# DakeQQ/Audio-Denoiser-ONNX

Measured on AMD Instinct MI355X. Metric: audio_seconds_per_second (GTCRN 16 kHz, batch=256 x 1 s chunks; RTF = 1/value), higher is better.
Workload: dtype f32; 1 GPU; GTCRN 16 kHz, batch=256 x 1 s chunks, fp32, int16 PCM in/out resident in HBM (BASELINE.json configs[1]); chunks_per_gpu=256, chunks_total=256, ranks=1, chunk_samples=16000, out_samples=15872, weights=seeded reference-architecture GTCRN (tests/golden/gtcrn_seed0.adew), stitch_all_gather=False

## Files before the change

audio_denoiser_onnx_amd/csrc/ade_engine.hip:

```cpp
#include "ade_internal.h"
#include "ade_gtcrn_pack.h"

#include "../../include/ade.h"

#if !defined(HIPSIM)
#include <dlfcn.h>
#endif

#include <algorithm>
#include <cmath>
#include <cstdio>
#include <cstdlib>
#include <cstring>
#include <map>
#include <mutex>
#include <string>
#include <vector>

using namespace ade;

namespace {

thread_local std::string g_create_error;

// ... 86 lines not shown
    int* d_ints = nullptr;
    FftTabs tabs{};
    BandTab erb_bm{}, erb_bs{};
    ConvW en0{}, en1{}, de3{}, de4{};
    GtConvW en_gt[3]{}, de_gt[3]{};
    DpW dp[2]{};

    int capacity = 0;
    int last_batch = 0;
    int16_t* d_pcm_in = nullptr;
    int16_t* d_pcm_out = nullptr;
    float* d_f32_out = nullptr;
    float* ws = nullptr;
    float *mean = nullptr, *spec = nullptr, *feat = nullptr, *e0 = nullptr, *e1 = nullptr, *h = nullptr, *zt = nullptr;
    float *xe[3] = {}, *ate[3] = {}, *xd[3] = {}, *atd[3] = {};
    float *rnn = nullptr, *dpm[2] = {}, *dpo[2] = {};
    float *d3 = nullptr, *mask = nullptr, *frames = nullptr;
    int16_t* h_pcm_in = nullptr;
    int16_t* h_pcm_out = nullptr;
    float* h_f32_out = nullptr;

    int stagger_ticks = 2750;
    int wave_swap = 0;
    int seg_prio = 0;
    int xwait_ticks = 20000000;
    int full_taps = 0;
    int xchg_withhold = 0;
    int xwait_retry = 1;
    bool timed_out = false;
    int retries = 0;
    int geometry = -1;
    ade::ChunkFixed* d_fixed = nullptr;
    float* d_xchg = nullptr;
    unsigned* d_xflags = nullptr;
    int* d_xerr = nullptr;
    int xl_B[kXErrWords] = {}, xl_chunk0[kXErrWords] = {};
    int xchg_capacity = 0;
    int xchg_segments = 0;
    bool use_graph = true;
    bool graph_supported = true;
    bool use_fused = true;
    bool use_single = true;
    bool last_fused = false;
    int last_geometry = -1;
    long long* d_clk = nullptr;
    std::vector<GraphEntry> graphs;
// ... 475 lines not shown
        hipEventRecord(e->events[cursor].second, s);
        ++cursor;
        e->events_used = cursor;
    }
};

int pick_geometry(const ade_engine* e, int ) {
    if (e->geometry >= 0) return fused_supported(e->T, e->geometry) ? e->geometry : -1;
    for (int g = fused_geometries() - 1; g >= 0; --g)
        if (fused_supported(e->T, g)) return g;
    return -1;
}

void enqueue(ade_engine* e, hipStream_t s, const int16_t* d_in, int B, int16_t* d_out, float* d_f32, bool prof) {
    const int T = e->T, nfr = B * T;
    Seq q{e, s, prof};
    const View none{nullptr, nullptr};
    const int geo = pick_geometry(e, B);
    const bool fused = e->use_fused && geo >= 0 && !e->gt_sand;
    e->last_fused = fused;
    View x{e->e1, nullptr};
    if (fused) {
        SegPlan plan{};
        plan.nseg = fused_segments(T, geo); plan.xchg = e->d_xchg; plan.flags = e->d_xflags; plan.err = e->d_xerr; plan.wave_swap = e->wave_swap;
        plan.prio = e->seg_prio;
        plan.withhold = e->xchg_withhold;
        plan.wait_ticks = e->xwait_ticks;
        e->last_geometry = geo;
        long long* clk = prof ? e->d_clk : nullptr;
        if (clk) (void)hipMemsetAsync(e->d_clk, 0, kClkSlots * sizeof(long long), s);
        const float* dc = nullptr;
        if (e->n_win > 1) {
            q.begin("pcm_mean"); launch_pcm_mean(s, d_in, B, e->in_len, e->mean, e->n_win); q.end();
            dc = e->mean;
        }
        if (e->use_single && (!prof || e->profile_mode >= 2)) {
            ChunkCall C{};
            C.fixed = e->d_fixed;
            C.dc = dc;
            C.stagger = (geo == 0 && B >= 192) ? e->stagger_ticks : 0;
            C.pcm_in = d_in; C.pcm_out = d_out; C.f32_out = d_f32; C.L = e->in_len; C.T = T; C.B = B;
            C.plan = plan;
            C.full_taps = e->full_taps;
            C.clk = (prof && e->profile_mode == 3) ? e->d_clk : nullptr;
            q.begin("gtcrn_chunk"); launch_gtcrn_chunk(s, geo, C); q.end();
            return;
        }
// ... 631 lines not shown
    d->max_batch = h->capacity / h->n_win;
    d->device = h->device;
    return ADE_OK;
}

ade_status ade_reserve(ade_handle h, int batch) {
    if (!h || batch < 0) return ADE_ERR_BAD_VALUE;
    return reserve(h, batch * h->n_win);
}

ade_status ade_set_option(ade_handle h, const char* key, const char* value) {
    if (!h || !key || !value) return ADE_ERR_BAD_VALUE;
    if (strcmp(key, "stagger_us") == 0) {
        char* end = nullptr;
        const double us = strtod(value, &end);
        if (!value[0] || *end || us < 0.0 || us > 1000.0) return fail(h, ADE_ERR_BAD_VALUE, "option stagger_us: 0..1000");
        h->stagger_ticks = (int)(us * 100.0 + 0.5);
        return ADE_OK;
    }
    if (strcmp(key, "wave_swap") == 0) {
        bool b;
        if (!parse_bool(value, &b)) return fail(h, ADE_ERR_BAD_VALUE, "option wave_swap must be 0/1");
        h->wave_swap = b;
        return ADE_OK;
    }
    if (strcmp(key, "seg_prio") == 0) {
        if (value[0] < '0' || value[0] > '4' || value[1]) return fail(h, ADE_ERR_BAD_VALUE, "option seg_prio: 0..4");
        h->seg_prio = value[0] - '0';
        return ADE_OK;
    }
    if (strcmp(key, "xwait_ms") == 0) {
        char* end = nullptr;
        const double ms = strtod(value, &end);
        if (!value[0] || *end || !(ms >= 0.001) || ms > 20000.0) return fail(h, ADE_ERR_BAD_VALUE, "option xwait_ms: 0.001..20000");
        h->xwait_ticks = (int)(ms * 1e5 + 0.5);
        if (h->sub) h->sub->set_exchange_wait_ticks(h->xwait_ticks);
        free_graphs(h);
        return ADE_OK;
    }
    if (strcmp(key, "pipe_depth") == 0) {
        if (value[0] < '2' || value[0] > '4' || value[1]) return fail(h, ADE_ERR_BAD_VALUE, "option pipe_depth: 2..4");
        for (const auto& sl : h->pipe) if (sl.state == 1) return fail(h, ADE_ERR_BAD_VALUE, "option pipe_depth: submissions are in flight (ade_wait them first)");
        h->pipe_depth = value[0] - '0';
        return ADE_OK;
    }
    if (strcmp(key, "xwait_retry") == 0) {
// ... 306 lines not shown
                    const std::string _what = std::string(#expr) + ": " + hipGetErrorString(_err);                           \
                    if (launched) {                                                                                          \
                        (void)hipStreamSynchronize(h->stream); (void)hipStreamSynchronize(h->s_in); (void)hipStreamSynchronize(h->s_out); \
                        (void)exchange_status(h, "ade_process", false);                                                      \
                        (void)hipGetLastError();                                                                             \
                    }                                                                                                        \
                    return fail(h, ADE_ERR_DEVICE, _what);                                                                   \
                }                                                                                                            \
            } while (0)
            const unsigned epoch = ++h->sio_epoch ? h->sio_epoch : ++h->sio_epoch;
            h->last_batch = rows;
            h->last_fused = true;
            h->last_geometry = geo;
            h->h_sio_epoch[0] = epoch;
            for (int g = 0; g < used; ++g) {
                const int r0 = g * per, nr = std::min(per, rows - r0);
                const size_t i0 = (size_t)r0 * h->in_len;
                const int16_t* src = in + i0;
                if (!in_direct) { memcpy(h->h_pcm_in + i0, in + i0, (size_t)nr * h->in_len * sizeof(int16_t)); src = h->h_pcm_in + i0; }
                SIO_TRY(hipMemcpyAsync(h->d_pcm_in + i0, src, (size_t)nr * h->in_len * sizeof(int16_t), hipMemcpyHostToDevice, h->s_in));
                SIO_TRY(hipMemcpyAsync(h->d_sio_ready + (size_t)g * kReadyStride, h->h_sio_epoch, (size_t)kReadyStride * sizeof(unsigned), hipMemcpyHostToDevice, h->s_in));
                if (g == 0) {
                    ChunkCall C{};
                    C.plan.nseg = fused_segments(h->T, geo); C.plan.xchg = h->d_xchg; C.plan.flags = h->d_xflags; C.plan.err = h->d_xerr; C.plan.wave_swap = h->wave_swap;
                    C.plan.prio = h->seg_prio; C.plan.withhold = h->xchg_withhold; C.plan.wait_ticks = h->xwait_ticks;
                    C.fixed = h->d_fixed;
                    C.pcm_in = h->d_pcm_in; C.pcm_out = h->d_pcm_out; C.f32_out = out_f32 ? h->d_f32_out : nullptr;
                    C.L = h->in_len; C.T = h->T; C.B = rows; C.chunk0 = 0;
                    C.full_taps = h->full_taps;
                    C.in_ready = h->d_sio_ready; C.out_done = h->h_sio_done; C.out_count = h->d_sio_count; C.epoch = epoch; C.group_rows = per;
                    launch_gtcrn_chunk(h->stream, geo, C);
                    launched = true;
                    SIO_TRY(hipGetLastError());
                }
            }
            volatile unsigned* const done = h->h_sio_done;
            bool finished = false;
            for (int g = 0; g < used; ++g) {
                const int r0 = g * per, nr = std::min(per, rows - r0);
                const size_t o0 = (size_t)r0 * h->out_len;
                for (unsigned spins = 0; done[g] != epoch && !finished; ++spins)
                    if ((spins & 0x3ffu) == 0x3ffu && hipStreamQuery(h->stream) == hipSuccess) finished = true;
                if (out_pcm) SIO_TRY(hipMemcpyAsync((pcm_direct ? out_pcm : h->h_pcm_out) + o0, h->d_pcm_out + o0, (size_t)nr * h->out_len * sizeof(int16_t), hipMemcpyDeviceToHost, h->s_out));
                if (out_f32) SIO_TRY(hipMemcpyAsync((f32_direct ? out_f32 : h->h_f32_out) + o0, h->d_f32_out + o0, (size_t)nr * h->out_len * sizeof(float), hipMemcpyDeviceToHost, h->s_out));
            }
#undef SIO_TRY
            (void)hipGetLastError();
// ... 12 lines not shown
        }
    }
    {
        const int geo = pick_geometry(h, rows);
        int n_sub = h->host_split ? h->host_split : (rows >= 128 ? 2 : 1);
        const bool plain = !h->sub && !h->gt_sand && h->use_fused && h->use_single && geo >= 0 && !h->profile && h->n_win == 1;
        if (plain && n_sub > 1 && rows >= 2 * n_sub) {
            const int per = (rows + n_sub - 1) / n_sub;
            h->last_batch = rows;
            h->last_fused = true;
            h->last_geometry = geo;
            const int used = (rows + per - 1) / per;
            for (int k = 0; k < used; ++k) {
                const int r0 = k * per, nr = std::min(per, rows - r0);
                if (!h->sub_streams[k]) HIP_TRY(h, hipStreamCreateWithFlags(&h->sub_streams[k], hipStreamNonBlocking));
                const size_t i0 = (size_t)r0 * h->in_len;
                const int16_t* src = in + i0;
                if (!in_direct) { memcpy(h->h_pcm_in + i0, in + i0, (size_t)nr * h->in_len * sizeof(int16_t)); src = h->h_pcm_in + i0; }
                HIP_TRY(h, hipMemcpyAsync(h->d_pcm_in + i0, src, (size_t)nr * h->in_len * sizeof(int16_t), hipMemcpyHostToDevice, h->sub_streams[k]));
            }
            for (int k = 0; k < used; ++k) {
                const int r0 = k * per, nr = std::min(per, rows - r0);
                ChunkCall C{};
                C.plan.nseg = fused_segments(h->T, geo); C.plan.xchg = h->d_xchg; C.plan.flags = h->d_xflags; C.plan.wave_swap = h->wave_swap;
                C.plan.err = h->d_xerr + k;
                h->xl_B[k] = nr; h->xl_chunk0[k] = r0;
                C.plan.prio = h->seg_prio; C.plan.withhold = r0 == 0 ? h->xchg_withhold : 0; C.plan.wait_ticks = h->xwait_ticks;
                C.fixed = h->d_fixed;
                C.pcm_in = h->d_pcm_in; C.pcm_out = h->d_pcm_out; C.f32_out = out_f32 ? h->d_f32_out : nullptr;
                C.L = h->in_len; C.T = h->T; C.B = nr; C.chunk0 = r0;
                C.full_taps = h->full_taps;
                launch_gtcrn_chunk(h->sub_streams[k], geo, C);
                HIP_TRY(h, hipGetLastError());
            }
            for (int k = 0; k < used; ++k) {
                const int r0 = k * per, nr = std::min(per, rows - r0);
                const size_t o0 = (size_t)r0 * h->out_len;
                hipStream_t s = h->sub_streams[k];
                if (out_pcm) HIP_TRY(h, hipMemcpyAsync((pcm_direct ? out_pcm : h->h_pcm_out) + o0, h->d_pcm_out + o0, (size_t)nr * h->out_len * sizeof(int16_t), hipMemcpyDeviceToHost, s));
                if (out_f32) HIP_TRY(h, hipMemcpyAsync((f32_direct ? out_f32 : h->h_f32_out) + o0, h->d_f32_out + o0, (size_t)nr * h->out_len * sizeof(float), hipMemcpyDeviceToHost, s));
            }
            for (int k = 0; k < used; ++k) HIP_TRY(h, hipStreamSynchronize(h->sub_streams[k]));
            st = exchange_status(h, "ade_process", false);
            for (int k = 0; k < kXErrWords; ++k) h->xl_B[k] = 0;
            if (st != ADE_OK) {
                if (out_pcm && pcm_direct) memset(out_pcm, 0, nout * sizeof(int16_t));
                if (out_f32 && f32_direct) memset(out_f32, 0, nout * sizeof(float));
// ... 639 lines not shown
```

audio_denoiser_onnx_amd/csrc/ade_fused.hip:

```cpp
#include "ade_stage_frontback.h"

namespace ade {

using namespace stage;

namespace {

constexpr size_t cmax(size_t a, size_t b) { return a > b ? a : b; }
template <class G> constexpr size_t chunk_smem_bytes() {
    return cmax(cmax(gt_smem_bytes<G>(), dp_smem_bytes<G>()), cmax(front_smem_bytes<G>(), back_smem_bytes<G>()));
}
static_assert(chunk_smem_bytes<Geo1>() * 2 <= 160 * 1024, "two geometry-1 workgroups must fit one CU's LDS");
static_assert(chunk_smem_bytes<Geo2>() * 4 <= 160 * 1024, "four geometry-2 workgroups must fit one CU's LDS");
static_assert(chunk_smem_bytes<Geo0>() <= 160 * 1024, "geometry 0 must fit one CU's LDS");

__device__ __forceinline__ Seg make_seg(const SegPlan& plan, int B, int T, int block, int& chunk, int chunk0 = 0) {
    const int seg = block / B;
    chunk = chunk0 + block - seg * B;
    const int base = T / plan.nseg, rem = T - base * plan.nseg;
    Seg sg;
    sg.T = T;
    sg.nT = base + (seg < rem ? 1 : 0);
    sg.t0 = seg * base + (seg < rem ? seg : rem);
    sg.prev = seg > 0;
    sg.next = seg + 1 < plan.nseg;
    sg.swap = plan.wave_swap && (seg & 1);
    sg.stream = plan.stream;
    const size_t slot = (size_t)chunk * plan.nseg + seg;
    sg.xo = plan.xchg + slot * kXFloats;
    sg.xi = plan.xchg + (slot - (seg > 0 ? 1 : 0)) * kXFloats;
    sg.fo = plan.flags + slot * kXFlags;
    sg.fi = plan.flags + (slot - (seg > 0 ? 1 : 0)) * kXFlags;
    sg.err = plan.err;
    if (seg == 0 && plan.carry_in) {
        sg.prev = 1;
        sg.xi = plan.carry_in + (size_t)chunk * kXFloats;
        sg.fi = plan.carry_in_flags + (size_t)chunk * kXFlags;
    }
    if (seg + 1 == plan.nseg && plan.carry_out) {
        sg.next = 1;
        sg.xo = plan.carry_out + (size_t)chunk * kXFloats;
        sg.fo = plan.carry_out_flags + (size_t)chunk * kXFlags;
    }
    if (plan.withhold && block == 0) sg.fo = plan.flags + ((size_t)B * plan.nseg - 1) * kXFlags;
    sg.first = !sg.prev;
    sg.base_prio = plan.prio == 4 ? (seg < 2 ? 2 - seg : 0) : (seg > 0 ? plan.prio : 0);
    return sg;
}
__device__ __forceinline__ long long* seg_clk(long long* clk, const Seg& sg, int B, int block) {
// ... 188 lines not shown
```

audio_denoiser_onnx_amd/csrc/ade_internal.h:

```cpp
#pragma once
#include <map>
#include <string>
#include <vector>

#include <hip/hip_runtime.h>

#include <cstddef>
#include <cstdint>

namespace ade {

constexpr int kNfft = 512;
constexpr int kHop = 256;
constexpr int kBins = 257;
constexpr int kBinsPad = 260;
constexpr int kErb = 129;
constexpr int kErbPad = 132;
constexpr int kErbLow = 65;
constexpr int kErbBands = 64;
constexpr int kErbHigh = 192;
constexpr int kF1 = 65;
constexpr int kFw = 33;
constexpr int kCh = 16;
constexpr int kTileFrames = 7;
// ... 88 lines not shown
                         float f32_scale, int nan_to_num );
void launch_half_to_float(hipStream_t s, const uint16_t* in, float* out, long long n);
void launch_float_to_half(hipStream_t s, const float* in, uint16_t* out, long long n);
void launch_ola_pcm_stream(hipStream_t s, const float* frames, float* carry, FftTabs tabs, int B, int T, bool first, int16_t* pcm, float* f32);

constexpr int kXHistFrames = 10;
constexpr int kXHistFloats = 4 * kXHistFrames * kFw * 4;
constexpr int kXTraOff = 6 * kXHistFloats;
constexpr int kXInterOff = kXTraOff + 6 * 16;
constexpr int kXOlaOff = kXInterOff + 2 * kFw * 16;
constexpr int kXPendOff = kXOlaOff + kHop;
constexpr int kXFloats = ((kXPendOff + kHop + 63) / 64) * 64;
constexpr int kXFlags = 16;
constexpr int kXFlagHist = 0, kXFlagTra = 6, kXFlagInter = 12, kXFlagOla = 14;
constexpr int kMaxSegments = 8;
constexpr int kClkSlotsPerSeg = 64 * 10;
struct SegPlan {
    int wait_ticks;
    int nseg;
    float* xchg;
    unsigned* flags;
    int* err;
    int wave_swap;
    float* carry_in;
    unsigned* carry_in_flags;
    float* carry_out;
    unsigned* carry_out_flags;
    int stream;
    int prio;
    int withhold;
};
struct Seg {
    int t0, nT, T;
    int prev, next;
    int swap;
    int stream;
    int first;
    int base_prio;
    float* xo;
    float* xi;
    unsigned* fo;
    unsigned* fi;
    int* err;
};
int fused_geometries();
int fused_max_frames(int geometry);
bool fused_supported(int T, int geometry);
int fused_segments(int T, int geometry);
hipError_t fused_init();
void launch_gtblock(hipStream_t s, int geometry, SegPlan plan, int blk, const float* a, const float* skip, GtConvW w, float* out, int B, int T, long long* clk);
void launch_dpgrnn(hipStream_t s, int geometry, SegPlan plan, int blk, const float* x, DpW w, float* out, int B, int T, long long* clk);
void launch_front(hipStream_t s, int geometry, SegPlan plan, const int16_t* pcm, int B, int L, int T, FftTabs tabs, BandTab erb_bm, ConvW c0, ConvW c1, float* spec,
                  float* e0, float* e1, long long* clk, const float* dc = nullptr);
void launch_back(hipStream_t s, int geometry, SegPlan plan, const float* x, const float* e1, const float* e0, const float* spec, ConvW c3, ConvW c4, BandTab erb_bs,
                 FftTabs tabs, int16_t* pcm, float* f32, int B, int T, long long* clk);

struct ChunkFixed {
    FftTabs tabs;
// ... 85 lines not shown
```

audio_denoiser_onnx_amd/csrc/ade_stage_frontback.h:

```cpp
#pragma once
#include "ade_stage_net.h"

namespace ade {
namespace stage {

constexpr int kWbuf = 264;
constexpr size_t kTabFloats = 512 + 2 * 256 + 2 * 264;
constexpr int kBmCap = 16;
constexpr int kBsCap = 4;

__device__ __forceinline__ float2 rfft_bin(float2 zk, float2 zp, float2 w) {
    const float2 e = make_float2(0.5f * (zk.x + zp.x), 0.5f * (zk.y - zp.y));
    const float2 d = make_float2(0.5f * (zk.x - zp.x), 0.5f * (zk.y + zp.y));
    const float2 o = make_float2(d.y, -d.x);
    return make_float2(e.x + (w.x * o.x - w.y * o.y), e.y + (w.x * o.y + w.y * o.x));
}

struct LdsTabs { const float* win; const float2* tw256; const float2* tw512; };
template <class G>
__device__ __forceinline__ LdsTabs stage_tables(float* dst, const FftTabs& t, int tid) {
    constexpr int kFusedThreads = G::kThreads;
    float* win = dst;
    float* tw256 = dst + 512;
    float* tw512 = tw256 + 512;
// ... 41 lines not shown
            (size_t)(G::kLean ? 0 : kBmCap) * kErbBands + kC0TailW + kC1TailW + 16) * 4;
}

template <class G>
__device__ __forceinline__ void front_stage(float* smem, int chunk, const Seg& sg, const int16_t* __restrict__ pcm, int L, const FftTabs& tabs,
                                            const BandTab& erb, const ConvW& c0, const ConvW& c1, float* __restrict__ spec,
                                            float* __restrict__ e0, float* __restrict__ e1, long long* __restrict__ clk,
                                            const float* __restrict__ dc_rows = nullptr) {
    constexpr int kFusedThreads = G::kThreads, kTileF = G::kTileF, kTileP1 = kTileF * kF1;
    constexpr size_t kFrontFeatFloats = (size_t)kTileF * 3 * kErb;
    constexpr int kGroupShift = (kFusedThreads == 1024 ? 9 : (kFusedThreads == 512 ? 8 : 7));
    static_assert(kFusedThreads == 1024 || kFusedThreads == 512 || kFusedThreads == 256, "front / back conv rounds: 64 lanes per frame");
    constexpr int kBmRows = G::kLean ? 0 : kBmCap;
    const int T = sg.T, tbeg = sg.t0, tend = sg.t0 + sg.nT;
    float2* wbuf_all = reinterpret_cast<float2*>(smem);
    float* feat = smem + kTileF * kWbuf * 2;
    float4* E0 = reinterpret_cast<float4*>(feat + kFrontFeatFloats);
    float* E0f = reinterpret_cast<float*>(E0);
    float* tabmem = reinterpret_cast<float*>(E0 + 4 * kTileP1);
    float* erbw = tabmem + kTabFloats;
    float* w0t = erbw + kBmRows * kErbBands;
    float* w1t = w0t + kC0TailW;
    int* red = reinterpret_cast<int*>(w1t + kC1TailW);
    int tid_ = threadIdx.x;
    ADE_OPAQUE_V(tid_);
    const int tid = tid_, wave = tid >> 6, lane = tid & 63;
    const int16_t* row = pcm + (size_t)chunk * L;
    const int P0 = T * kF1, P = T * kFw;
    float* e0c = e0 + (size_t)chunk * kCh * P0;
    float* e1c = e1 + (size_t)chunk * kCh * P;
    float* specc = spec + (size_t)chunk * T * 2 * kBinsPad;
    ADE_CLK(32);
    const bool pair_ok = ((L & 1) == 0) && ((reinterpret_cast<size_t>(row) & 3) == 0);
    int raw[4];
    const int centre = sg.stream ? 0 : kNfft / 2;
    load_frame_pairs(row, L, tbeg + wave, lane, tbeg + wave < tend, pair_ok, raw, centre);
    const LdsTabs lt = stage_tables<G>(tabmem, tabs, tid);
    const bool erb_lds = erb.count <= kBmRows;
    if (erb_lds)
        for (int i = tid; i < erb.count * kErbBands; i += kFusedThreads) erbw[i] = erb.w[i];
    const int erb_s0 = erb.start[lane];
    for (int i = tid; i < kC0TailW; i += kFusedThreads) w0t[i] = c0.w[i];
    for (int i = tid; i < kC1TailW; i += kFusedThreads) w1t[i] = c1.w[i];
    const float b0t = c0.b[tid & 15], b1t = c1.b[tid & 15];

    if (!dc_rows) {
        int s = 0;
        if (((L & 7) == 0) && ((reinterpret_cast<size_t>(row) & 15) == 0)) {
            const int4* r4 = reinterpret_cast<const int4*>(row);
#pragma unroll 2
            for (int i = tid; i < (L >> 3); i += kFusedThreads) {
                const int4 q = r4[i];
                s += (int)(short)(q.x & 0xffff) + (q.x >> 16) + (int)(short)(q.y & 0xffff) + (q.y >> 16)
                   + (int)(short)(q.z & 0xffff) + (q.z >> 16) + (int)(short)(q.w & 0xffff) + (q.w >> 16);
            }
        } else {
            for (int i = tid; i < L; i += kFusedThreads) s += (int)row[i];
        }
#pragma unroll
        for (int off = 32; off >= 1; off >>= 1) s += __shfl_xor(s, off);
        if (lane == 0) red[wave] = s;
    }
    __syncthreads();
    float dc;
    if (dc_rows) {
        dc = dc_rows[chunk];
    } else {
        long long tot = 0;
#pragma unroll
        for (int i = 0; i < kTileF; ++i) tot += red[i];
        dc = (float)((double)tot / ((double)L * 32768.0));
    }
    ADE_CLK(33);
    long long clk_prev = ADE_CLK_START();
    const cfptr c0b = cptr(c0.b), c1b = cptr(c1.b);
    const cfptr c0e = cptr(c0.w) + 5 * 9 * 16;

    for (int t0 = tbeg; t0 < tend; t0 += kTileF) {
        const int nf = tend - t0 < kTileF ? tend - t0 : kTileF;
        {
            int tq = tid;
            ADE_OPAQUE_V(tq);
            const int wave = tq >> 6, lane = tq & 63;
            float2* buf = wbuf_all + wave * kWbuf;
            const int t = t0 + wave;
            const bool live = wave < nf;
            float2 v[4];
#pragma unroll
            for (int r = 0; r < 4; ++r) {
                const int n = lane + 64 * r;
                const float sa = (float)(short)(raw[r] & 0xffff) * (1.0f / 32768.0f) - dc;
                const float sb = (float)(raw[r] >> 16) * (1.0f / 32768.0f) - dc;
                v[r] = make_float2(sa * lt.win[2 * n], sb * lt.win[2 * n + 1]);
            }
            {
                const int tn = t + kTileF;
                load_frame_pairs(row, L, tn, lane, tn < tend, pair_ok, raw, centre);
            }
            fft256_inplace(v, buf, lane, lt.tw256);
            wave_sync();
#pragma unroll
            for (int r = 0; r < 4; ++r) buf[lane + 64 * r] = v[r];
            wave_sync();
            {
                float2 xa[2], xb[2];
#pragma unroll
                for (int r = 0; r < 2; ++r) {
                    const int k = lane + 64 * r;
                    const float2 zk = buf[k], zp = buf[(256 - k) & 255];
                    xa[r] = rfft_bin(zk, zp, lt.tw512[k]);
                    xb[r] = rfft_bin(zp, zk, lt.tw512[256 - k]);
                }
                float2 xm = make_float2(0.0f, 0.0f);
                if (lane == 0) { const float2 z = buf[128]; xm = rfft_bin(z, z, lt.tw512[128]); }
                wave_sync();
#pragma unroll
                for (int r = 0; r < 2; ++r) {
                    const int k = lane + 64 * r;
                    buf[k] = xa[r];
                    buf[256 - k] = xb[r];
                }
                if (lane == 0) buf[128] = xm;
            }
            wave_sync();
            if (live) {
                float* fr = feat + (size_t)wave * 3 * kErb;
#pragma unroll
                for (int r = 0; r < 5; ++r) {
                    if (r == 4 && lane != 0) break;
                    const int k = r < 4 ? lane + 64 * r : 256;
                    const float2 x = buf[k];
                    specc[((size_t)t * 2 + 0) * kBinsPad + k] = x.x;
                    specc[((size_t)t * 2 + 1) * kBinsPad + k] = x.y;
                    if (k < kErbLow) {
                        fr[k] = fast_sqrt((x.x * x.x + x.y * x.y) + 1e-12f);
                        fr[kErb + k] = x.x;
                        fr[2 * kErb + k] = x.y;
                    }
                }
                if (erb_lds) erb_merge(erbw, erb.count, erb_s0, buf, lane, fr);
                else erb_merge(erb.w, erb.count, erb_s0, buf, lane, fr);
            }
        }
        __syncthreads();
        ADE_CLK(34);
        ADE_CLK_ACC(40);
        {
            int tq = tid;
            ADE_OPAQUE_V(tq);
            const int tl = tq >> 6, g = (tq >> 4) & 3, j = tq & 15;
            if (tl < nf) {
                const float* fr = feat + (size_t)tl * 3 * kErb;
                float wa[6];
#pragma unroll
                for (int kk = 0; kk < 6; ++kk) wa[kk] = c0e[((kk >> 1) * 8 + 4 * (kk & 1) + g) * 16 + j];
                v4f cb;
#pragma unroll
                for (int r = 0; r < 4; ++r) cb[r] = c0b[4 * g + r];
                const float sel0 = prelu_sel(c0.slope);
#pragma unroll
                for (int mt = 0; mt < 4; ++mt) {
                    const int fo = 16 * mt + j;
                    const int q0 = 2 * fo - 3 + g;
                    const bool v0 = q0 >= 0;
// ... 111 lines not shown
    static_assert((size_t)4 * kTileP * 4 >= (size_t)kTileF * kWbuf * 2, "the S tile must be able to hold the FFT buffers");
    static_assert((size_t)4 * kTileP1 * 4 >= kBackAccFloats, "the D tile must be able to hold the overlap-add accumulator");
    constexpr int kSUnits = 4 * kTileP;
    constexpr int kSThreads = kSUnits / 3;
    static_assert(kSThreads * 3 == kSUnits && kSThreads <= kFusedThreads, "S staging split");
    constexpr int kGroupShift = (kFusedThreads == 1024 ? 9 : (kFusedThreads == 512 ? 8 : 7));
    constexpr bool kLean = G::kLean;
    const int T = sg.T, tbeg = sg.t0, tend = sg.t0 + sg.nT;
    float4* S = reinterpret_cast<float4*>(smem);
    float* Sf = smem;
    float2* wbuf_all = reinterpret_cast<float2*>(smem);
    float4* D = S + 4 * kTileP;
    float* Df = reinterpret_cast<float*>(D);
    float* M = reinterpret_cast<float*>(D + 4 * kTileP1);
    float* acc = Df;
    float* cbuf = M + kTileF * 2 * kErbPad;
    float* tabmem = cbuf + kHop;
    float* bsw = tabmem + kTabFloats;
    float* w3t = bsw + kBsCap * kErbHigh;
    float* w4t = w3t + kC3TailW;
    float* wsum = kLean ? const_cast<float*>(tabs.win_sum) : w4t + kC4TailW;
    int* bss = reinterpret_cast<int*>(wsum + kHop);
    float* pend = kLean ? sg.xo + kXPendOff : reinterpret_cast<float*>(bss + kErbHigh);
    int tid_ = threadIdx.x;
    ADE_OPAQUE_V(tid_);
    const int tid = tid_;
    const int P0 = T * kF1, P = T * kFw;
    const float* xc = x + (size_t)chunk * kCh * P;
    const float* e1c = e1 + (size_t)chunk * kCh * P;
    const float* e0c = e0 + (size_t)chunk * kCh * P0;
    const float* specc = spec + (size_t)chunk * T * 2 * kBinsPad;
    const int trim = sg.stream ? 0 : kHop;
    const int out_len = sg.stream ? kHop * T : kHop * (T - 1);
    int16_t* po = pcm ? pcm + (size_t)chunk * out_len : nullptr;
    float* fo32 = f32 ? f32 + (size_t)chunk * out_len : nullptr;
    ADE_CLK(48);

    auto issue_s = [&](int t0n, bool go, float4* sa, float4* sb) {
        const int nfn = tend - t0n < kTileF ? tend - t0n : kTileF;
        int tq = tid;
        ADE_OPAQUE_V(tq);
        const bool on = go && tq < kSThreads;
#pragma unroll
        for (int i = 0; i < 3; ++i) {
            const int u = tq + kSThreads * i, q = u / kTileP, idx = u - q * kTileP;
            const int idc = idx < nfn * kFw ? idx : 0;
            const size_t off = ((size_t)q * P + (size_t)t0n * kFw + idc) * 4;
// ... 170 lines not shown
                }
            }
        }
        if (tid < kTileF * 2) {
            const int tl = tid >> 1, co = tid & 1;
            if (tl < nf) {
                float ev = b4t;
#pragma unroll
                for (int dlt = -1; dlt <= 0; ++dlt) {
                    const int ps = tl * kF1 + (kF1 - 1) + dlt;
#pragma unroll
                    for (int ci = 0; ci < 16; ++ci)
                        ev += w4t[(dlt < 0 ? 32 : 0) + ci * 2 + co] * Df[((size_t)(ci >> 2) * kTileP1 + ps) * 4 + (ci & 3)];
                }
                M[(size_t)tl * 2 * kErbPad + co * kErbPad + (kErb - 1)] = tanh_f(ev);
            }
        }
        __syncthreads();
        ADE_CLK(51);
        ADE_CLK_ACC(58);
        {
            int tq = tid;
            ADE_OPAQUE_V(tq);
            const int wave = tq >> 6, lane = tq & 63;
            float2* buf = wbuf_all + wave * kWbuf;
            const bool live = wave < nf;
            const float* mr = M + (size_t)(live ? wave : 0) * 2 * kErbPad;
#pragma unroll
            for (int r = 0; r < 5; ++r) {
                if (r == 4 && lane != 0) break;
                const int k = r < 4 ? lane + 64 * r : 256;
                const float xr = sre[r], xi = sim[r];
                float m0, m1;
                if (k < kErbLow) {
                    m0 = mr[k];
                    m1 = mr[kErbPad + k];
                } else {
                    const int o = k - kErbLow;
                    m0 = 0.0f; m1 = 0.0f;
                    if (bs_lds) {
                        const int s0 = kLean ? bs_s[r > 0 ? r - 1 : 0] : bss[o];
                        for (int n = 0; n < bs.count; ++n) {
                            const float wv = bsw[n * kErbHigh + o];
                            const int jj = min(s0 + n, kErbBands - 1);
                            m0 += mr[kErbLow + jj] * wv;
                            m1 += mr[kErbPad + kErbLow + jj] * wv;
                        }
                    } else {
                        const int s0 = bs.start[o];
                        for (int n = 0; n < bs.count; ++n) {
                            const float wv = bs.w[n * kErbHigh + o];
                            const int jj = min(s0 + n, kErbBands - 1);
                            m0 += mr[kErbLow + jj] * wv;
                            m1 += mr[kErbPad + kErbLow + jj] * wv;
                        }
                    }
                }
                float2 y = make_float2(__fmaf_rn(xr, m0, -(xi * m1)), __fmaf_rn(xi, m0, xr * m1));
                if (k == 0 || k == 256) y.y = 0.0f;
                buf[k] = y;
            }
            wave_sync();
            float2 v[4];
#pragma unroll
            for (int r = 0; r < 4; ++r) {
                const int k = lane + 64 * r;
                const float2 yk = buf[k], yp = buf[256 - k];
                const float2 e = make_float2(0.5f * (yk.x + yp.x), 0.5f * (yk.y - yp.y));
                const float2 d = make_float2(0.5f * (yk.x - yp.x), 0.5f * (yk.y + yp.y));
                const float2 o = fcmul(d, make_float2(lt.tw512[k].x, -lt.tw512[k].y));
                v[r] = make_float2(e.x - o.y, -(e.y + o.x));
            }
            wave_sync();
            fft256_inplace(v, buf, lane, lt.tw256);
            const bool park = sg.prev && t0 == tbeg && wave == 0;
#pragma unroll
            for (int par = 0; par < 2; ++par) {
                if (live && (wave & 1) == par) {
#pragma unroll
                    for (int r = 0; r < 4; ++r) {
                        const int n = lane + 64 * r;
                        const float pa = v[r].x * (1.0f / 256.0f), pb = -v[r].y * (1.0f / 256.0f);
                        float wa = pa * lt.win[2 * n], wb = pb * lt.win[2 * n + 1];
                        ADE_OPAQUE_V(wa);
                        ADE_OPAQUE_V(wb);
                        float2* a = reinterpret_cast<float2*>(acc + kHop * wave + 2 * n);
                        if (park && r < 2) {
                            *reinterpret_cast<float2*>(pend + 2 * n) = make_float2(wa, wb);
                        } else if (par == 0) {
                            float2 c = make_float2(0.0f, 0.0f);
                            if (wave == 0 && r < 2) c = *reinterpret_cast<const float2*>(cbuf + 2 * n);
                            *a = make_float2(c.x + wa, c.y + wb);
                        } else if (r < 2 || wave + 1 < nf) {
                            float2 c = *a;
                            c.x += wa;
                            c.y += wb;
                            *a = c;
// ... 75 lines not shown
```

audio_denoiser_onnx_amd/csrc/ade_stage_net.h:

```cpp
#pragma once
#include "ade_device.h"

#include <type_traits>

#ifndef ADE_DP_INTER_MFMA
#define ADE_DP_INTER_MFMA 0
#endif

namespace ade {
namespace stage {

using namespace dev;


template <int NT, int TMAX, int WAVES_PER_SIMD>
struct Geo {
    static constexpr int kThreads = NT;
    static constexpr int kWavesPerSimd = WAVES_PER_SIMD;
    static constexpr int kTmax = TMAX;
    static constexpr int kPmax = TMAX * kFw;
    static constexpr int kPosPerThread = (kPmax + NT - 1) / NT;
    static constexpr int kTileF = NT / 64;
    static constexpr int kProdBase = ((TMAX * (kFw / 3) + 63) / 64) * 64;
    static constexpr bool kLean = NT < 512;
    static_assert(kPosPerThread == 3, "the conv phases are written for three positions per lane");
    static_assert(kProdBase < NT, "the history producers need a wavefront outside the conv lanes");
};
typedef Geo<1024, 64, 4> Geo0;
typedef Geo<512, 32, 4> Geo1;
typedef Geo<256, 16, 4> Geo2;

__device__ __forceinline__ float comp(const float4& v, int c) { return c == 0 ? v.x : (c == 1 ? v.y : (c == 2 ? v.z : v.w)); }

__device__ __forceinline__ void pl_ld8(const float* Xc, int P, int p, int q0, float* v) {
    ld4(Xc + ((size_t)q0 * P + p) * 4, v);
    ld4(Xc + ((size_t)(q0 + 1) * P + p) * 4, v + 4);
}
__device__ __forceinline__ void pl_ld16(const float* Xc, int P, int p, float* v) {
    pl_ld8(Xc, P, p, 0, v);
    pl_ld8(Xc, P, p, 2, v + 8);
}
__device__ __forceinline__ void pl_st16(float* Xc, int P, int p, const float* v) {
#pragma unroll
    for (int q = 0; q < 4; ++q) st4(Xc + ((size_t)q * P + p) * 4, v + 4 * q);
}

template <class G> constexpr size_t gt_smem_bytes() { return (size_t)4 * G::kPmax * 16 + 2 * G::kTmax * 8 * 4; }

#define ADE_REP16(M) M(0) M(1) M(2) M(3) M(4) M(5) M(6) M(7) M(8) M(9) M(10) M(11) M(12) M(13) M(14) M(15)

#define ADE_CLK(i) do { if (clk && chunk == 0 && threadIdx.x == 0) clk[i] = wall_clock64(); } while (0)
#define ADE_CLK_START() ((clk && chunk == 0 && threadIdx.x == 0) ? wall_clock64() : 0)
#define ADE_CLK_ACC(i) do { if (clk && chunk == 0 && threadIdx.x == 0) { const long long n_ = wall_clock64(); clk[i] += n_ - clk_prev; clk_prev = n_; } } while (0)

template <class G>
__device__ __forceinline__ void gtblock_stage(float4* smem, int chunk, const Seg& sg, int blk, const float* __restrict__ a, const float* __restrict__ skip,
                                              const GtConvW& w, float* __restrict__ out, long long* __restrict__ clk,
                                              bool x1_in_lds = false, bool next_x1 = false, const float* __restrict__ next_skip = nullptr, bool store_lo = true,
                                              bool next_full = false) {
    constexpr int kFusedThreads = G::kThreads, kTmaxFused = G::kTmax, kPmax = G::kPmax, kPosPerThread = G::kPosPerThread;
    float4* H = smem;
    float* zt = reinterpret_cast<float*>(smem + 4 * kPmax);
    float* at = zt + kTmaxFused * 8;
    float* GI = reinterpret_cast<float*>(smem + 2 * kPmax);
    float* HS = GI + kTmaxFused * 48;
    const int T = sg.nT;
    const int P = T * kFw;
    const int Ps = sg.T * kFw;
    int tid_ = threadIdx.x;
    if (kFusedThreads == 512 && sg.swap) tid_ ^= (tid_ & 256) >> 1;
    ADE_OPAQUE_V(tid_);
    const int tid = tid_;
    const size_t cbase = (size_t)chunk * kCh * Ps + (size_t)sg.t0 * kFw * 4;
    const float* ac = a + cbase;
    const float* sc = skip ? skip + cbase : nullptr;
    float* oc = out + cbase;
    const cfptr c_pw1_b = cptr(w.pw1_b), c_dw_b = cptr(w.dw_b), c_pw2_b = cptr(w.pw2_b);
    cfptr c_pw1, c_dw, c_pw2;
    ADE_SCALAR_COPY(c_pw1, cptr(w.pw1));
    ADE_SCALAR_COPY(c_dw, cptr(w.dw));
    ADE_SCALAR_COPY(c_pw2, cptr(w.pw2));
    const float pw1_slope = w.pw1_slope, dw_slope = w.dw_slope;
    const float pw1_sel = prelu_sel(pw1_slope), dw_sel = prelu_sel(dw_slope);
    const int dilation = w.dilation;
    ADE_CLK(0);

    if (!x1_in_lds) {
        constexpr int kIt = (kPmax + kFusedThreads - 1) / kFusedThreads;
        float x[kIt][8], y[kIt][8];
#pragma unroll
        for (int i = 0; i < kIt; ++i) {
            const int p = tid + i * kFusedThreads, pc = p < P ? p : P - 1;
            pl_ld8(ac, Ps, pc, 0, x[i]);
            if (sc) pl_ld8(sc, Ps, pc, 0, y[i]);
        }
#pragma unroll
        for (int i = 0; i < kIt; ++i) {
            const int p = tid + i * kFusedThreads;
            if (p >= P) break;
            if (sc) {
#pragma unroll
                for (int k = 0; k < 8; ++k) x[i][k] += y[i][k];
            }
            H[2 * kPmax + p] = make_float4(x[i][0], x[i][1], x[i][2], x[i][3]);
            H[3 * kPmax + p] = make_float4(x[i][4], x[i][5], x[i][6], x[i][7]);
        }
        __syncthreads();
    }
    constexpr int kWaves = kFusedThreads / 64;
    constexpr int kTiles = (kPmax / 16 + kWaves - 1) / kWaves;
    static_assert(kPmax % 16 == 0, "whole tiles");
    const int wave = __builtin_amdgcn_readfirstlane(tid >> 6);
    const int g = (tid >> 4) & 3, jn = tid & 15;
    const float* Hf = reinterpret_cast<const float*>(H);
    const char* const Hb = reinterpret_cast<const char*>(H);
    constexpr int kZ0 = 4 * kPmax * 16;
    constexpr int kPairs = (kTiles + 1) / 2;
    float4 hi[kPairs];
    {
        float wa[2][6];
#pragma unroll
        for (int kk = 0; kk < 6; ++kk) {
            wa[0][kk] = c_pw1[((4 * (kk & 1) + g) * 3 + (kk >> 1)) * 16 + jn];
            wa[1][kk] = c_pw1[((4 * (kk & 1) + g) * 3 + (kk >> 1)) * 16 + (jn ^ 8)];
        }
        v4f cb[2];
#pragma unroll
        for (int r = 0; r < 4; ++r) { cb[0][r] = c_pw1_b[4 * g + r]; cb[1][r] = c_pw1_b[(4 * g + r) ^ 8]; }
#pragma unroll
        for (int it = 0; it < kTiles; ++it) {
            const int od = it & 1;
            const int pu = (it * kWaves + wave) * 16 + jn, pos = pu < P ? pu : P - 1;
            const int f = pos - (pos / kFw) * kFw;
            const bool lok = f != 0, rok = f != kFw - 1;
            const char* xb = Hb + (pos * 4 + g) * 4;
            v4f d = cb[od];
#pragma unroll
            for (int kk = 0; kk < 6; ++kk) {
                const int o = kk >> 1;
                float x = *reinterpret_cast<const float*>(xb + ((2 + (kk & 1)) * kPmax + (o - 1)) * 16);
                if (o == 0) x = lok ? x : 0.0f;
                if (o == 2) x = rok ? x : 0.0f;
                d = mfma16x16x4(wa[od][kk], x, d);
            }
            const v2f d0 = mk2(d[0], d[1]), d1 = mk2(d[2], d[3]);
            const v2f a0 = d0 * mk2(pw1_slope, pw1_slope), a1 = d1 * mk2(pw1_slope, pw1_slope);
            const float4 r4 = make_float4(prelu_m(d0[0], a0[0], pw1_sel), prelu_m(d0[1], a0[1], pw1_sel),
                                          prelu_m(d1[0], a1[0], pw1_sel), prelu_m(d1[1], a1[1], pw1_sel));
            const bool now = (g < 2) != (od != 0);
            if (now && pu < P) H[(g & 1) * kPmax + pu] = r4;
            if (!od) {
                hi[it >> 1] = r4;
            } else {
                hi[it >> 1] = make_float4(now ? hi[it >> 1].x : r4.x, now ? hi[it >> 1].y : r4.y, now ? hi[it >> 1].z : r4.z, now ? hi[it >> 1].w : r4.w);
            }
        }
    }
    __syncthreads();
#pragma unroll
    for (int pr = 0; pr < kPairs; ++pr) {
        const int it = 2 * pr + (g < 2 ? 1 : 0);
        const int pu = (it * kWaves + wave) * 16 + jn;
        if (it < kTiles && pu < P) H[(2 + (g & 1)) * kPmax + pu] = hi[pr];
    }
    if (tid < 12) zt[tid] = 0.0f;
    if (sg.prev && tid == 0) xwait(sg.fi + kXFlagHist + blk, sg.err, xcode(kXFlagHist + blk));
    __syncthreads();
    ADE_CLK(1);

    float4 h1r[kPairs];
    {
        v2f wd[3][3][2];
#pragma unroll
        for (int kt = 0; kt < 3; ++kt)
#pragma unroll
            for (int kf = 0; kf < 3; ++kf) {
                const int o = kt * 48 + kf * 16 + 4 * g;
                wd[kt][kf][0] = mk2(c_dw[o], c_dw[o + 1]);
                wd[kt][kf][1] = mk2(c_dw[o + 2], c_dw[o + 3]);
            }
        const v2f db0 = mk2(c_dw_b[4 * g], c_dw_b[4 * g + 1]), db1 = mk2(c_dw_b[4 * g + 2], c_dw_b[4 * g + 3]);
        const int dstep = dilation * kFw * 16;
        const char* const zp = Hb + kZ0;
// ... 34 lines not shown
                    acc0 = mk2(v.x, v.y);
                    acc1 = mk2(v.z, v.w);
                }
                dw_taps(acc0, acc1, j, f, pn + P, 2);
                if (pu < NP) xst4(xhist_o, (g * kXHistFrames * kFw + pn) * 4, make_float4(acc0[0], acc0[1], acc1[0], acc1[1]));
            }
            xdrain();
            __syncthreads();
            if (tid == 0) xflag_store(sg.fo + kXFlagHist + blk, 1u);
        }
        float wp[2][4];
#pragma unroll
        for (int r = 0; r < 4; ++r) {
            const float wv = c_pw2[(4 * g + r) * 8 + (jn & 7)];
            wp[0][r] = jn < 8 ? wv : 0.0f;
            wp[1][r] = jn < 8 ? 0.0f : wv;
        }
        v4f cb2;
#pragma unroll
        for (int r = 0; r < 4; ++r) cb2[r] = c_pw2_b[(4 * g + r) & 7];
        v4f d2 = cb2;
#pragma unroll
        for (int it = 0; it < kTiles; ++it) {
            const int pu = (it * kWaves + wave) * 16 + jn, pos = pu < P ? pu : P - 1;
            const int t = pos / kFw, f = pos - t * kFw;
            v2f acc0 = db0, acc1 = db1;
            if (sg.prev && (it * kWaves + wave) * 16 < NP) {
                const float4 v = xld4(xhist_i, (g * kXHistFrames * kFw + (pos < NP ? pos : NP - 1)) * 4);
                const bool head = pos < NP;
                acc0 = mk2(head ? v.x : db0[0], head ? v.y : db0[1]);
                acc1 = mk2(head ? v.z : db1[0], head ? v.w : db1[1]);
            }
            dw_taps(acc0, acc1, t, f, pos, 3);
            const v2f a0 = acc0 * mk2(dw_slope, dw_slope), a1 = acc1 * mk2(dw_slope, dw_slope);
            const float y[4] = {prelu_m(acc0[0], a0[0], dw_sel), prelu_m(acc0[1], a0[1], dw_sel),
                                prelu_m(acc1[0], a1[0], dw_sel), prelu_m(acc1[1], a1[1], dw_sel)};
            if (!(it & 1)) d2 = cb2;
#pragma unroll
            for (int r = 0; r < 4; ++r) d2 = mfma16x16x4(wp[it & 1][r], y[r], d2);
            if ((it & 1) || it == kTiles - 1) h1r[it >> 1] = make_float4(d2[0], d2[1], d2[2], d2[3]);
        }
    }
    __syncthreads();
    ADE_CLK(2);
#pragma unroll
    for (int pr = 0; pr < kPairs; ++pr) {
        const int it = 2 * pr + (g >> 1);
        const int pu = (it * kWaves + wave) * 16 + jn;
        if (it < kTiles && pu < P) H[(g & 1) * kPmax + pu] = h1r[pr];
    }
    __syncthreads();
    ADE_CLK(3);

    v2f wr_raw[8];
    float bh_raw = 0.0f;
    {
        const int j = tid & 15, row = (tid >> 4) & 3;
        const int gsel = (row & 1) ? 2 : (row >> 1);
        const float* pk = w.gru + j * 78 + 24 + gsel * 16;
#pragma unroll
        for (int m = 0; m < 8; ++m) wr_raw[m] = tid < 64 ? mk2(pk[2 * m], pk[2 * m + 1]) : mk2(0.0f, 0.0f);
        if (tid < 64) bh_raw = w.gru[j * 78 + 75 + gsel];
    }
    const float* nsc = (next_x1 && next_skip) ? next_skip + cbase : nullptr;
    float nsk[kPosPerThread][8];
    auto request_next_skip = [&]() {
#pragma unroll
        for (int i = 0; i < kPosPerThread; ++i) {
            const int p = tid + i * kFusedThreads;
// ... 112 lines not shown
            gi = gnx;
        }
        set_prio(sg.base_prio);
        if (sg.next) {
            if (row == 3) xst1(sg.xo + kXTraOff + blk * 16 + j, hv);
            xdrain();
            if (tid == 48) xflag_store(sg.fo + kXFlagTra + blk, 1u);
        }
    }
    __syncthreads();
    ADE_CLK(6);
    for (int idx = tid; idx < T * 8; idx += kFusedThreads) {
        const int t = idx >> 3, c = idx & 7;
        const float* fr = w.fc + c * 17;
        float s = fr[16];
#pragma unroll
        for (int k = 0; k < 16; ++k) s += fr[k] * HS[t * 16 + k];
        at[idx] = sigmoid_f(s);
    }
    __syncthreads();
    ADE_CLK(7);
#pragma unroll
    for (int pr = 0; pr < kPairs; ++pr) {
        const int it = 2 * pr + (g >> 1);
        const int pu = (it * kWaves + wave) * 16 + jn;
        if (it < kTiles && pu < P) {
            const float4 gt = *reinterpret_cast<const float4*>(at + (pu / kFw) * 8 + 4 * (g & 1));
            H[(2 + (g & 1)) * kPmax + pu] = make_float4(h1r[pr].x * gt.x, h1r[pr].y * gt.y, h1r[pr].z * gt.z, h1r[pr].w * gt.w);
        }
    }
    __syncthreads();
    float n8[kPosPerThread][8];
#pragma unroll
    for (int i = 0; i < kPosPerThread; ++i) {
        const int p = tid + i * kFusedThreads;
        if (p < P) {
            const float4 b0 = H[p], b1 = H[kPmax + p], g0 = H[2 * kPmax + p], g1 = H[3 * kPmax + p];
            const float o[16] = {g0.x, b0.x, g0.y, b0.y, g0.z, b0.z, g0.w, b0.w, g1.x, b1.x, g1.y, b1.y, g1.z, b1.z, g1.w, b1.w};
            if (store_lo) {
                pl_st16(oc, Ps, p, o);
            } else {
                st4(oc + ((size_t)2 * Ps + p) * 4, o + 8);
                st4(oc + ((size_t)3 * Ps + p) * 4, o + 12);
            }
#pragma unroll
            for (int k = 0; k < 8; ++k) n8[i][k] = o[k] + nsk[i][k];
// ... 96 lines not shown
    {
        const float ye = (de * rstd * ln_w[32 * kCh + j] + ln_b[32 * kCh + j]) + re;
        if (live) emit_one(p2, j, ye);
    }
}

__device__ __forceinline__ float gru_gates(const v4f& d, float h) {
    const float r = fast_rcp(1.0f + __builtin_amdgcn_exp2f(d[0]));
    const float z = fast_rcp(1.0f + __builtin_amdgcn_exp2f(d[1]));
    const float n = 1.0f - 2.0f * fast_rcp(__builtin_amdgcn_exp2f(d[3] + r * d[2]) + 1.0f);
    return n + z * (h - n);
}

template <class G>
__device__ __forceinline__ void dpgrnn_stage(float4* smem, int chunk, const Seg& sg, int blk, const float* __restrict__ x, const DpW& w, float* __restrict__ out,
                                             long long* __restrict__ clk, bool next_x1 = false,
                                             const float* __restrict__ next_skip = nullptr, bool store_lo = true, bool x_in_lds = false, bool next_full = false) {
    constexpr int kFusedThreads = G::kThreads, kTmaxFused = G::kTmax, kPmax = G::kPmax, kPosPerThread = G::kPosPerThread;
    float4* R = smem;
    float* Rf = reinterpret_cast<float*>(smem);
    float* lnt = reinterpret_cast<float*>(smem + 4 * kPmax);
    const int T = sg.nT;
    const int P = T * kFw, Ps = sg.T * kFw;
    int tid_ = threadIdx.x;
    ADE_OPAQUE_V(tid_);
    const int tid = tid_;
    for (int i = tid; i < kFw * kCh; i += kFusedThreads) {
        lnt[i] = w.intra_ln_w[i];
        lnt[kFw * kCh + i] = w.intra_ln_b[i];
    }
    const size_t cbase = (size_t)chunk * kCh * Ps + (size_t)sg.t0 * kFw * 4;
    const float* xc = x + cbase;
    float* oc = out + cbase;

    ADE_CLK(16);
    {
        constexpr float kS = -kLog2e, kN = 2.0f * kLog2e;
        if (!x_in_lds) {
            float4 v[kPosPerThread][4];
#pragma unroll
            for (int i = 0; i < kPosPerThread; ++i) {
                const int p = tid + i * kFusedThreads, pc = p < P ? p : P - 1;
#pragma unroll
                for (int q = 0; q < 4; ++q) v[i][q] = *reinterpret_cast<const float4*>(xc + ((size_t)q * Ps + pc) * 4);
            }
#pragma unroll
            for (int i = 0; i < kPosPerThread; ++i) {
// ... 310 lines not shown
```

Before: 760,800 audio-s/s.

## Add wave rotation option, prefetch DC-sum loads, and skip dead tiles in fused stages

```diff
diff --git a/audio_denoiser_onnx_amd/csrc/ade_engine.hip b/audio_denoiser_onnx_amd/csrc/ade_engine.hip
--- a/audio_denoiser_onnx_amd/csrc/ade_engine.hip
+++ b/audio_denoiser_onnx_amd/csrc/ade_engine.hip
@@ -132,6 +132,7 @@
 
     int stagger_ticks = 2750;
     int wave_swap = 0;
+    int wave_rot = 0;
     int seg_prio = 0;
     int xwait_ticks = 20000000;
     int full_taps = 0;
@@ -653,7 +654,7 @@
     View x{e->e1, nullptr};
     if (fused) {
         SegPlan plan{};
-        plan.nseg = fused_segments(T, geo); plan.xchg = e->d_xchg; plan.flags = e->d_xflags; plan.err = e->d_xerr; plan.wave_swap = e->wave_swap;
+        plan.nseg = fused_segments(T, geo); plan.xchg = e->d_xchg; plan.flags = e->d_xflags; plan.err = e->d_xerr; plan.wave_swap = e->wave_swap; plan.wave_rot = e->wave_rot;
         plan.prio = e->seg_prio;
         plan.withhold = e->xchg_withhold;
         plan.wait_ticks = e->xwait_ticks;
@@ -1331,6 +1332,12 @@
         bool b;
         if (!parse_bool(value, &b)) return fail(h, ADE_ERR_BAD_VALUE, "option wave_swap must be 0/1");
         h->wave_swap = b;
+        return ADE_OK;
+    }
+    if (strcmp(key, "wave_rot") == 0) {
+        if (value[0] < '0' || value[0] > '4' || value[1]) return fail(h, ADE_ERR_BAD_VALUE, "option wave_rot: 0..4");
+        h->wave_rot = value[0] - '0';
+        free_graphs(h);
         return ADE_OK;
     }
     if (strcmp(key, "seg_prio") == 0) {
@@ -1683,7 +1690,7 @@
                 SIO_TRY(hipMemcpyAsync(h->d_sio_ready + (size_t)g * kReadyStride, h->h_sio_epoch, (size_t)kReadyStride * sizeof(unsigned), hipMemcpyHostToDevice, h->s_in));
                 if (g == 0) {
                     ChunkCall C{};
-                    C.plan.nseg = fused_segments(h->T, geo); C.plan.xchg = h->d_xchg; C.plan.flags = h->d_xflags; C.plan.err = h->d_xerr; C.plan.wave_swap = h->wave_swap;
+                    C.plan.nseg = fused_segments(h->T, geo); C.plan.xchg = h->d_xchg; C.plan.flags = h->d_xflags; C.plan.err = h->d_xerr; C.plan.wave_swap = h->wave_swap; C.plan.wave_rot = h->wave_rot;
                     C.plan.prio = h->seg_prio; C.plan.withhold = h->xchg_withhold; C.plan.wait_ticks = h->xwait_ticks;
                     C.fixed = h->d_fixed;
                     C.pcm_in = h->d_pcm_in; C.pcm_out = h->d_pcm_out; C.f32_out = out_f32 ? h->d_f32_out : nullptr;
@@ -1742,7 +1749,7 @@
             for (int k = 0; k < used; ++k) {
                 const int r0 = k * per, nr = std::min(per, rows - r0);
                 ChunkCall C{};
-                C.plan.nseg = fused_segments(h->T, geo); C.plan.xchg = h->d_xchg; C.plan.flags = h->d_xflags; C.plan.wave_swap = h->wave_swap;
+                C.plan.nseg = fused_segments(h->T, geo); C.plan.xchg = h->d_xchg; C.plan.flags = h->d_xflags; C.plan.wave_swap = h->wave_swap; C.plan.wave_rot = h->wave_rot;
                 C.plan.err = h->d_xerr + k;
                 h->xl_B[k] = nr; h->xl_chunk0[k] = r0;
                 C.plan.prio = h->seg_prio; C.plan.withhold = r0 == 0 ? h->xchg_withhold : 0; C.plan.wait_ticks = h->xwait_ticks;
diff --git a/audio_denoiser_onnx_amd/csrc/ade_fused.hip b/audio_denoiser_onnx_amd/csrc/ade_fused.hip
--- a/audio_denoiser_onnx_amd/csrc/ade_fused.hip
+++ b/audio_denoiser_onnx_amd/csrc/ade_fused.hip
@@ -25,6 +25,7 @@
     sg.prev = seg > 0;
     sg.next = seg + 1 < plan.nseg;
     sg.swap = plan.wave_swap && (seg & 1);
+    sg.rot = plan.wave_rot == 1 ? ((seg + chunk) & 3) : (plan.wave_rot > 1 ? ((plan.wave_rot - 1) & 3) : 0);
     sg.stream = plan.stream;
     const size_t slot = (size_t)chunk * plan.nseg + seg;
     sg.xo = plan.xchg + slot * kXFloats;
diff --git a/audio_denoiser_onnx_amd/csrc/ade_internal.h b/audio_denoiser_onnx_amd/csrc/ade_internal.h
--- a/audio_denoiser_onnx_amd/csrc/ade_internal.h
+++ b/audio_denoiser_onnx_amd/csrc/ade_internal.h
@@ -134,6 +134,7 @@
     unsigned* flags;
     int* err;
     int wave_swap;
+    int wave_rot;
     float* carry_in;
     unsigned* carry_in_flags;
     float* carry_out;
@@ -146,6 +147,7 @@
     int t0, nT, T;
     int prev, next;
     int swap;
+    int rot;
     int stream;
     int first;
     int base_prio;
diff --git a/audio_denoiser_onnx_amd/csrc/ade_stage_frontback.h b/audio_denoiser_onnx_amd/csrc/ade_stage_frontback.h
--- a/audio_denoiser_onnx_amd/csrc/ade_stage_frontback.h
+++ b/audio_denoiser_onnx_amd/csrc/ade_stage_frontback.h
@@ -87,7 +87,7 @@
     float* w0t = erbw + kBmRows * kErbBands;
     float* w1t = w0t + kC0TailW;
     int* red = reinterpret_cast<int*>(w1t + kC1TailW);
-    int tid_ = threadIdx.x;
+    int tid_ = wave_tid<G>(sg);
     ADE_OPAQUE_V(tid_);
     const int tid = tid_, wave = tid >> 6, lane = tid & 63;
     const int16_t* row = pcm + (size_t)chunk * L;
@@ -100,6 +100,20 @@
     int raw[4];
     const int centre = sg.stream ? 0 : kNfft / 2;
     load_frame_pairs(row, L, tbeg + wave, lane, tbeg + wave < tend, pair_ok, raw, centre);
+    constexpr int kDcAhead = 8;
+    const bool dc_fast = !dc_rows && ((L & 7) == 0) && ((reinterpret_cast<size_t>(row) & 15) == 0);
+    const int dc_n = L >> 3;
+    int4 dq[kDcAhead];
+#pragma unroll
+    for (int k = 0; k < kDcAhead; ++k) dq[k].x = dq[k].y = dq[k].z = dq[k].w = 0;
+    if (dc_fast) {
+        const int4* r4 = reinterpret_cast<const int4*>(row);
+#pragma unroll
+        for (int k = 0; k < kDcAhead; ++k) {
+            const int i = tid + k * kFusedThreads;
+            dq[k] = r4[i < dc_n ? i : dc_n - 1];
+        }
+    }
     const LdsTabs lt = stage_tables<G>(tabmem, tabs, tid);
     const bool erb_lds = erb.count <= kBmRows;
     if (erb_lds)
@@ -111,10 +125,17 @@
 
     if (!dc_rows) {
         int s = 0;
-        if (((L & 7) == 0) && ((reinterpret_cast<size_t>(row) & 15) == 0)) {
+        if (dc_fast) {
             const int4* r4 = reinterpret_cast<const int4*>(row);
+#pragma unroll
+            for (int k = 0; k < kDcAhead; ++k) {
+                const int4 q = dq[k];
+                const int v = (int)(short)(q.x & 0xffff) + (q.x >> 16) + (int)(short)(q.y & 0xffff) + (q.y >> 16)
+                            + (int)(short)(q.z & 0xffff) + (q.z >> 16) + (int)(short)(q.w & 0xffff) + (q.w >> 16);
+                s += tid + k * kFusedThreads < dc_n ? v : 0;
+            }
 #pragma unroll 2
-            for (int i = tid; i < (L >> 3); i += kFusedThreads) {
+            for (int i = tid + kDcAhead * kFusedThreads; i < dc_n; i += kFusedThreads) {
                 const int4 q = r4[i];
                 s += (int)(short)(q.x & 0xffff) + (q.x >> 16) + (int)(short)(q.y & 0xffff) + (q.y >> 16)
                    + (int)(short)(q.z & 0xffff) + (q.z >> 16) + (int)(short)(q.w & 0xffff) + (q.w >> 16);
@@ -146,10 +167,11 @@
         {
             int tq = tid;
             ADE_OPAQUE_V(tq);
-            const int wave = tq >> 6, lane = tq & 63;
+            const int wave = __builtin_amdgcn_readfirstlane(tq >> 6), lane = tq & 63;
             float2* buf = wbuf_all + wave * kWbuf;
             const int t = t0 + wave;
             const bool live = wave < nf;
+            if (live) {
             float2 v[4];
 #pragma unroll
             for (int r = 0; r < 4; ++r) {
@@ -188,7 +210,7 @@
                 if (lane == 0) buf[128] = xm;
             }
             wave_sync();
-            if (live) {
+            {
                 float* fr = feat + (size_t)wave * 3 * kErb;
 #pragma unroll
                 for (int r = 0; r < 5; ++r) {
@@ -205,6 +227,7 @@
                 }
                 if (erb_lds) erb_merge(erbw, erb.count, erb_s0, buf, lane, fr);
                 else erb_merge(erb.w, erb.count, erb_s0, buf, lane, fr);
+            }
             }
         }
         __syncthreads();
@@ -362,7 +385,7 @@
     float* wsum = kLean ? const_cast<float*>(tabs.win_sum) : w4t + kC4TailW;
     int* bss = reinterpret_cast<int*>(wsum + kHop);
     float* pend = kLean ? sg.xo + kXPendOff : reinterpret_cast<float*>(bss + kErbHigh);
-    int tid_ = threadIdx.x;
+    int tid_ = wave_tid<G>(sg);
     ADE_OPAQUE_V(tid_);
     const int tid = tid_;
     const int P0 = T * kF1, P = T * kFw;
@@ -579,10 +602,12 @@
         {
             int tq = tid;
             ADE_OPAQUE_V(tq);
-            const int wave = tq >> 6, lane = tq & 63;
+            const int wave = __builtin_amdgcn_readfirstlane(tq >> 6), lane = tq & 63;
             float2* buf = wbuf_all + wave * kWbuf;
             const bool live = wave < nf;
             const float* mr = M + (size_t)(live ? wave : 0) * 2 * kErbPad;
+            float2 v[4] = {make_float2(0.0f, 0.0f), make_float2(0.0f, 0.0f), make_float2(0.0f, 0.0f), make_float2(0.0f, 0.0f)};
+            if (live) {
 #pragma unroll
             for (int r = 0; r < 5; ++r) {
                 if (r == 4 && lane != 0) break;
@@ -618,7 +643,6 @@
                 buf[k] = y;
             }
             wave_sync();
-            float2 v[4];
 #pragma unroll
             for (int r = 0; r < 4; ++r) {
                 const int k = lane + 64 * r;
@@ -630,6 +654,7 @@
             }
             wave_sync();
             fft256_inplace(v, buf, lane, lt.tw256);
+            }
             const bool park = sg.prev && t0 == tbeg && wave == 0;
 #pragma unroll
             for (int par = 0; par < 2; ++par) {
diff --git a/audio_denoiser_onnx_amd/csrc/ade_stage_net.h b/audio_denoiser_onnx_amd/csrc/ade_stage_net.h
--- a/audio_denoiser_onnx_amd/csrc/ade_stage_net.h
+++ b/audio_denoiser_onnx_amd/csrc/ade_stage_net.h
@@ -3,6 +3,9 @@
 
 #include <type_traits>
 
+#ifndef ADE_GT_GUARD_FROM
+#define ADE_GT_GUARD_FROM 0
+#endif
 #ifndef ADE_DP_INTER_MFMA
 #define ADE_DP_INTER_MFMA 0
 #endif
@@ -30,6 +33,13 @@
 typedef Geo<512, 32, 4> Geo1;
 typedef Geo<256, 16, 4> Geo2;
 
+template <class G>
+__device__ __forceinline__ int wave_tid(const Seg& sg) {
+    int t = threadIdx.x;
+    if (G::kThreads == 256) t ^= sg.rot << 6;
+    return t;
+}
+
 __device__ __forceinline__ float comp(const float4& v, int c) { return c == 0 ? v.x : (c == 1 ? v.y : (c == 2 ? v.z : v.w)); }
 
 __device__ __forceinline__ void pl_ld8(const float* Xc, int P, int p, int q0, float* v) {
@@ -49,9 +59,9 @@
 
 #define ADE_REP16(M) M(0) M(1) M(2) M(3) M(4) M(5) M(6) M(7) M(8) M(9) M(10) M(11) M(12) M(13) M(14) M(15)
 
-#define ADE_CLK(i) do { if (clk && chunk == 0 && threadIdx.x == 0) clk[i] = wall_clock64(); } while (0)
-#define ADE_CLK_START() ((clk && chunk == 0 && threadIdx.x == 0) ? wall_clock64() : 0)
-#define ADE_CLK_ACC(i) do { if (clk && chunk == 0 && threadIdx.x == 0) { const long long n_ = wall_clock64(); clk[i] += n_ - clk_prev; clk_prev = n_; } } while (0)
+#define ADE_CLK(i) do { if (clk && chunk == 0 && tid == 0) clk[i] = wall_clock64(); } while (0)
+#define ADE_CLK_START() ((clk && chunk == 0 && tid == 0) ? wall_clock64() : 0)
+#define ADE_CLK_ACC(i) do { if (clk && chunk == 0 && tid == 0) { const long long n_ = wall_clock64(); clk[i] += n_ - clk_prev; clk_prev = n_; } } while (0)
 
 template <class G>
 __device__ __forceinline__ void gtblock_stage(float4* smem, int chunk, const Seg& sg, int blk, const float* __restrict__ a, const float* __restrict__ skip,
@@ -67,7 +77,7 @@
     const int T = sg.nT;
     const int P = T * kFw;
     const int Ps = sg.T * kFw;
-    int tid_ = threadIdx.x;
+    int tid_ = wave_tid<G>(sg);
     if (kFusedThreads == 512 && sg.swap) tid_ ^= (tid_ & 256) >> 1;
     ADE_OPAQUE_V(tid_);
     const int tid = tid_;
@@ -113,6 +123,7 @@
     const int wave = __builtin_amdgcn_readfirstlane(tid >> 6);
     const int g = (tid >> 4) & 3, jn = tid & 15;
     const float* Hf = reinterpret_cast<const float*>(H);
+    auto tile_live = [&](int it) { return it < ADE_GT_GUARD_FROM || (it * kWaves + wave) * 16 < P; };
     const char* const Hb = reinterpret_cast<const char*>(H);
     constexpr int kZ0 = 4 * kPmax * 16;
     constexpr int kPairs = (kTiles + 1) / 2;
@@ -129,6 +140,7 @@
         for (int r = 0; r < 4; ++r) { cb[0][r] = c_pw1_b[4 * g + r]; cb[1][r] = c_pw1_b[(4 * g + r) ^ 8]; }
 #pragma unroll
         for (int it = 0; it < kTiles; ++it) {
+            if (!tile_live(it)) continue;
             const int od = it & 1;
             const int pu = (it * kWaves + wave) * 16 + jn, pos = pu < P ? pu : P - 1;
             const int f = pos - (pos / kFw) * kFw;
@@ -159,6 +171,7 @@
     __syncthreads();
 #pragma unroll
     for (int pr = 0; pr < kPairs; ++pr) {
+        if (!tile_live(2 * pr)) continue;
         const int it = 2 * pr + (g < 2 ? 1 : 0);
         const int pu = (it * kWaves + wave) * 16 + jn;
         if (it < kTiles && pu < P) H[(2 + (g & 1)) * kPmax + pu] = hi[pr];
@@ -239,6 +252,7 @@
         v4f d2 = cb2;
 #pragma unroll
         for (int it = 0; it < kTiles; ++it) {
+            if (tile_live(it)) {
             const int pu = (it * kWaves + wave) * 16 + jn, pos = pu < P ? pu : P - 1;
             const int t = pos / kFw, f = pos - t * kFw;
             v2f acc0 = db0, acc1 = db1;
@@ -255,6 +269,7 @@
             if (!(it & 1)) d2 = cb2;
 #pragma unroll
             for (int r = 0; r < 4; ++r) d2 = mfma16x16x4(wp[it & 1][r], y[r], d2);
+            }
             if ((it & 1) || it == kTiles - 1) h1r[it >> 1] = make_float4(d2[0], d2[1], d2[2], d2[3]);
         }
     }
@@ -262,6 +277,7 @@
     ADE_CLK(2);
 #pragma unroll
     for (int pr = 0; pr < kPairs; ++pr) {
+        if (!tile_live(2 * pr)) continue;
         const int it = 2 * pr + (g >> 1);
         const int pu = (it * kWaves + wave) * 16 + jn;
         if (it < kTiles && pu < P) H[(g & 1) * kPmax + pu] = h1r[pr];
@@ -420,6 +436,7 @@
     ADE_CLK(7);
 #pragma unroll
     for (int pr = 0; pr < kPairs; ++pr) {
+        if (!tile_live(2 * pr)) continue;
         const int it = 2 * pr + (g >> 1);
         const int pu = (it * kWaves + wave) * 16 + jn;
         if (it < kTiles && pu < P) {
@@ -562,7 +579,7 @@
     float* lnt = reinterpret_cast<float*>(smem + 4 * kPmax);
     const int T = sg.nT;
     const int P = T * kFw, Ps = sg.T * kFw;
-    int tid_ = threadIdx.x;
+    int tid_ = wave_tid<G>(sg);
     ADE_OPAQUE_V(tid_);
     const int tid = tid_;
     for (int i = tid; i < kFw * kCh; i += kFusedThreads) {
```

After: 750,300 audio-s/s. 0.986x the previous value.
